# facebookresearch/Active-3D-Vision-and-Touch

Hardware: AMD Instinct MI355X
Metric: mesh-recon iters/sec (fwd+bwd, 2562-vert GCN + 10k-pt Chamfer) at bs=64 (higher is better)
Workload: dtype f32; 1 GPU; icosphere-4 template (2562 verts, 5120 faces), 3-stage GCN 20x300 cut 0.33, bs=64/GPU, 10000-pt Chamfer x3 draws, Adam, ellipsoid clouds (BASELINE.json configs[1]); global_batch=64, parallelism=dp1

## Files before the change

active-3d-vision-and-touch_amd/csrc/capi.hip:

```cpp
#include <stdarg.h>
#include <stdlib.h>
#include <string.h>

#include "../../include/a3vt.h"
#include <atomic>
#include <mutex>
#include <unordered_map>

#include "kernels.h"
#include "prims.h"

namespace a3vt {

static thread_local char g_err[512] = "";

void set_error(const char *fmt, ...) {
  va_list ap;
  va_start(ap, fmt);
  vsnprintf(g_err, sizeof(g_err), fmt, ap);
  va_end(ap);
}

__device__ float g_zero_page[64];
static const float *zero_page() {
// ... 35 lines not shown
static Prof g_prof;

struct ProfScope {
  int slot = -1;
  hipStream_t s;
  ProfScope(int cls, hipStream_t stream, bool timed = true) : s(stream) {
    if (!timed || !g_prof.on || g_prof.used >= Prof::kMax) return;
    slot = g_prof.used++;
    if (slot >= g_prof.created) {
      (void)hipEventCreate(&g_prof.ev[slot][0]);
      (void)hipEventCreate(&g_prof.ev[slot][1]);
      g_prof.created = slot + 1;
    }
    g_prof.cls[slot] = cls;
    (void)hipEventRecord(g_prof.ev[slot][0], s);
  }
  ~ProfScope() {
    if (slot >= 0) (void)hipEventRecord(g_prof.ev[slot][1], s);
  }
};

struct StackLayout {
  size_t wt, wt_stride;
  size_t za;
  int ldza;
  size_t z3;
  size_t ping[2];
  size_t panel;
  size_t dw_slab, db_slab, thin_dw_slab, thin_db_slab;
  size_t db_layer_stride;
  size_t heavy;
  size_t gq;
  size_t ell;
  size_t total;
};

constexpr int kQuadCols = 160;
static std::atomic<long long> g_path_counts[PATH_COUNT];
void path_count(int which) { g_path_counts[which].fetch_add(1, std::memory_order_relaxed); }
static int g_csr_algo = 0;
static SplitRef split_ref(const a3vt_adj_split *sp) {
  return sp ? SplitRef{sp->rowptr, sp->col, sp->scale, sp->cls} : SplitRef{nullptr, nullptr, nullptr, nullptr};
}
static bool split_whole(const a3vt_adj_split *sp) {
  const SplitRef r = split_ref(sp);
  return !sp || (r.rowptr && r.col && r.scale && r.cls);
}
static bool split_usable(const a3vt_adj_split *sp, int n_vert, int cut_len) {
  return sp && sp->max_degree > 0 && sp->max_degree <= csrqs_max_degree() && csrqs_fits(n_vert, cut_len);
}
static bool use_csrq(int batch, int n_vert, int hidden, int cut_len, int mode, int max_degree) {
  if (mode == GEMM_BF16_OPERANDS || mode == GEMM_BF16_STORAGE) return false;
  if (g_csr_algo != 2 && (max_degree <= 0 || max_degree > csrq_max_degree())) return false;
  if (g_csr_algo == 1 || cut_len <= 0) return false;
  return hidden % 4 == 0 && hidden >= kQuadCols + 16 && csrq_fits(n_vert, cut_len) && dw_quad_major_ok(hidden, kQuadCols / 4) &&
         rowgemm_quad_major_ok(batch * n_vert, hidden, pad4(cut_len));
}
static std::mutex g_stash_mu;
static std::unordered_map<const void *, int> g_stash_layout;
static void stash_layout_record(const void *masks, bool quad) {
  if (!masks) return;
  std::lock_guard<std::mutex> lock(g_stash_mu);
  if (g_stash_layout.size() > 4096) g_stash_layout.clear();
  g_stash_layout[masks] = quad ? 1 : 0;
}
static int stash_layout_lookup(const void *masks) {
  std::lock_guard<std::mutex> lock(g_stash_mu);
  auto it = g_stash_layout.find(masks);
  return it == g_stash_layout.end() ? -1 : it->second;
}
static int reduce_bias_partials(const float *slab, size_t layer_stride, int nslab, int cpad, int cut_len, int hidden, int last,
                                float *const *grad_biases, int acc, hipStream_t s) {
  for (int i0 = 0; i0 < last; i0 += kMaxImages) {
// ... 60 lines not shown
  bool x3;
  int omode;
  bool quad;
  bool qsplit;
  int qcols;
  int rm_ld;
  size_t rm_off;
};
static StackPlan stack_plan(int mode, int batch, int n_vert, int hidden, int num_layers, int cut_len, int max_degree,
                            const a3vt_adj_split *split, int rec) {
  StackPlan p{};
  const size_t m = (size_t)batch * n_vert;
  p.x3 = mode == GEMM_FP32X3 && num_layers > 2 && rowgemm3_stack_ok((long long)m, hidden, mask_ld(hidden, cut_len));
  p.omode = mode == GEMM_BF16_OPERANDS ? GEMM_BF16_OPERANDS : GEMM_FP32;
  const bool split_ok = split_usable(split, n_vert, cut_len);
  p.quad = num_layers > 1 &&
           (rec >= 0 ? rec == 1 : use_csrq(batch, n_vert, hidden, cut_len, mode, split_ok ? csrq_max_degree() : max_degree));
  p.qsplit = p.quad && split_ok;
  p.qcols = p.quad ? kQuadCols : 0;
  p.rm_ld = hidden - p.qcols;
  p.rm_off = m * p.qcols;
  return p;
}

static int launch_stack_ell(const StackPlan &p, const a3vt_adj_split *split, const int32_t *rowptr, const int32_t *col,
                            const float *val, int n_vert, int32_t *ell, hipStream_t s) {
  if (p.qsplit) {
    const SplitRef r = split_ref(split);
    return launch_csrqs_image(r.rowptr, r.col, r.scale, r.cls, n_vert, ell, s);
  }
  return p.quad ? launch_csrq_ell(rowptr, col, val, n_vert, ell, s) : 0;
}

static StackLayout stack_layout(int batch, int n_vert, int in_features, int hidden, int num_layers, int cut_len,
                                int need_backward, int gemm_mode = 0) {
  StackLayout L{};
  const size_t m = (size_t)batch * n_vert;
  const int cpad = pad4(cut_len);
  Arena a;
  const int kmax = hidden > pad4(in_features) ? hidden : pad4(in_features);
  L.wt_stride = align_up((size_t)rowgemm_bt_rows(kmax) * pad16(kmax), 64);
  if (gemm_mode == GEMM_FP32X3 && L.wt_stride < 3 * (size_t)kX3ImageFloats) L.wt_stride = 3 * (size_t)kX3ImageFloats;
  L.wt = a.take(L.wt_stride * (num_layers > 1 ? num_layers - 1 : 1));
  L.ldza = cpad > 4 ? cpad : 4;
  L.za = a.take(m * L.ldza);
  L.z3 = a.take(2 * m * 4);
  L.ping[0] = a.take(m * hidden);
  L.ping[1] = a.take(m * hidden);
  L.heavy = a.take(csr_heavy_scratch_ints(n_vert));
  L.ell = a.take(csrq_ell_ints(n_vert));
  if (need_backward) {
    const size_t kin = kmax;
    L.panel = a.take(pad4(in_features) > 304 ? m * 300 : 0);
    L.dw_slab = a.take((size_t)dw_slab_capacity(hidden) * kin * hidden);
    const size_t nslab = (size_t)csr_bwd_num_slabs(batch, n_vert) > (size_t)batch ? csr_bwd_num_slabs(batch, n_vert) : batch;
    L.db_layer_stride = align_up(nslab * cpad, 64);
    L.db_slab = a.take(L.db_layer_stride * (num_layers > 1 ? num_layers - 1 : 1));
    L.gq = a.take(m * L.ldza);
    L.thin_dw_slab = a.take((size_t)thin_num_slabs() * kin * 3);
    L.thin_db_slab = a.take((size_t)thin_num_slabs() * 3);
  }
  L.total = a.off;
  return L;
}

static int dw_panels(DwArgs d, const float *x, int ldx, int kin, float *panel, float *grad, int acc, bool timed, hipStream_t s) {
  const int cblk = kin > 304 ? 300 : kin;
  for (int c0 = 0; c0 < kin; c0 += cblk) {
    const int w = kin - c0 < cblk ? kin - c0 : cblk;
    d.x = x;
    d.ldx = ldx;
    if (kin > 304) {
      if (pad4(w) != w) { set_error("gcn_stack: in_features=%d needs a multiple of 4 past 300", kin); return -1; }
      if (int rc = launch_copy_cols(x, ldx, c0, w, panel, (long long)d.m, s)) return rc;
      d.x = panel;
      d.ldx = w;
    }
    d.k_in = w;
    {
      ProfScope ps(PROF_DW, s, timed);
      if (int rc = launch_dw(d, s)) return rc;
    }
    const size_t n = (size_t)w * d.n_out;
    if (int rc = launch_slab_reduce_za(d.slab, dw_images(d), n, n, n, grad + (size_t)c0 * d.n_out, acc, s)) return rc;
  }
  return 0;
}

static int check_stack_dims(int ld_feats, int in_features, int num_layers, int hidden, int cut_len) {
  if (num_layers < 1) { set_error("gcn_stack: num_layers=%d", num_layers); return -1; }
  if (ld_feats != pad4(in_features)) {
    set_error("gcn_stack: ld_feats=%d must be in_features=%d rounded up to a multiple of 4", ld_feats, in_features);
    return -1;
// ... 576 lines not shown
                           float *const *grad_biases, float *grad_feats, float *scratch, int accumulate, void *stream) {
  const int acc = accumulate ? 1 : 0;
  const float *acts = static_cast<const float *>(acts_v);
  (void)biases; (void)rowptr; (void)col; (void)val;
  A3VT_CHECK_ARG(feats && weights && rowptrT && colT && valT && grad_update && grad_weights && grad_biases);
  A3VT_CHECK_ARG(grad_feats && scratch && n_vert > 0 && batch > 0 && split_whole(split));
  A3VT_CHECK_ARG(gemm_bf16 >= GEMM_FP32 && gemm_bf16 <= GEMM_FP32X3);
  A3VT_CHECK_ARG(num_layers == 1 || acts != nullptr);
  A3VT_CHECK_ARG(num_layers <= 2 || masks != nullptr);
  if (int rc = check_stack_dims(ld_feats, in_features, num_layers, hidden, cut_len)) return rc;
  hipStream_t s = static_cast<hipStream_t>(stream);
  if (gemm_bf16 == GEMM_BF16_STORAGE)
    return stack_bwd16(feats, ld_feats, in_features, weights, num_layers, hidden, cut_len, rowptrT, colT, valT,
                       max_degreeT, split, n_vert, batch, acts, masks, grad_update, grad_weights, grad_biases, grad_feats,
                       scratch, acc, s);
  const float *zeros = zero_page();
  A3VT_CHECK_ARG(zeros != nullptr);
  const StackLayout L = stack_layout(batch, n_vert, in_features, hidden, num_layers, cut_len, 1, gemm_bf16);
  const StackStash S = stack_stash(batch, n_vert, hidden, num_layers, cut_len, gemm_bf16);
  const size_t m = (size_t)batch * n_vert;
  const int cpad = pad4(cut_len);
  const int last = num_layers - 1;

  const SplitRef sref = split_ref(split);
  int32_t *heavyT;
  if (int rc = hub_rows(rowptrT, n_vert, max_degreeT, scratch + L.heavy, &heavyT, s)) return rc;
  const StackPlan P = stack_plan(gemm_bf16, batch, n_vert, hidden, num_layers, cut_len, max_degreeT, split,
                                 masks ? stash_layout_lookup(masks) : 0);
  const bool quad = P.quad;
  const int qcols = P.qcols, rm_ld = P.rm_ld;
  const size_t rm_off = P.rm_off;
  int32_t *ellT = reinterpret_cast<int32_t *>(scratch + L.ell);
  if (int rc = launch_stack_ell(P, split, rowptrT, colT, valT, n_vert, ellT, s)) return rc;
  {
    const float *xl = num_layers == 1 ? feats : acts + S.act(last - 1);
    const float *x = xl + rm_off - qcols;
    const int ldx = num_layers == 1 ? ld_feats : rm_ld;
    const int k = num_layers == 1 ? in_features : hidden;
    float *gprev = num_layers == 1 ? grad_feats : scratch + L.ping[0];
    const int ldg = num_layers == 1 ? ld_feats : hidden;
    ProfScope pso(PROF_OUT, s);
    if (int rc = launch_thin_bwd(x, ldx, k, weights[last], rowptrT, colT, valT, heavyT, n_vert, batch, grad_update,
                                 scratch + L.z3, num_layers > 1, gprev, ldg, ldg, scratch + L.thin_dw_slab,
                                 scratch + L.thin_db_slab, quad ? scratch + L.gq : nullptr, cpad / 4, quad ? xl : nullptr,
                                 qcols / 4, s, split ? &sref : nullptr))
      return rc;
    if (int rc = reduce_output_grads(scratch + L.thin_dw_slab, scratch + L.thin_db_slab, k, grad_weights[last], grad_biases[last],
                                     acc, s))
      return rc;
  }

  if (P.x3)
    if (int rc = launch_stack_images(GEMM_FP32X3, 0, weights, 1, last, in_features, hidden, ld_feats, hidden, scratch + L.wt,
                                     L.wt_stride, s))
      return rc;
  if (int rc = launch_stack_images(GEMM_FP32, 0, weights, 0, P.x3 ? 1 : last, in_features, hidden, ld_feats, hidden,
                                   scratch + L.wt, L.wt_stride, s))
    return rc;

  const int db_rows = quad ? batch : csr_bwd_num_slabs(batch, n_vert);
  int cur = 0;
  for (int i = last - 1; i >= 0; --i) {
    float *g = scratch + L.ping[cur];
    float *dza = scratch + L.za;
    const float *xl = i == 0 ? feats : acts + S.act(i - 1);
    const bool xhyb = quad && i > 0;
    const float *x = xhyb ? xl + rm_off - qcols : xl;
    const int ldx = i == 0 ? ld_feats : (xhyb ? rm_ld : hidden);
    const int kin = i == 0 ? in_features : hidden;

    if (cut_len > 0 && quad) {
      const uint8_t *sq = masks + S.signq(i);
      ProfScope psa(PROF_AGG, s);
      if (P.qsplit) {
        if (int rc = launch_csrqs_bwd(scratch + L.gq, cut_len, ellT, n_vert, batch, dza, sq,
                                      scratch + L.db_slab + (size_t)i * L.db_layer_stride, s))
          return rc;
      } else if (int rc = launch_csrq_bwd(scratch + L.gq, cut_len, rowptrT, colT, valT, heavyT, ellT, n_vert, batch, dza, sq,
                                          scratch + L.db_slab + (size_t)i * L.db_layer_stride, s)) {
        return rc;
      }
    } else if (cut_len > 0) {
      ProfScope psa(PROF_AGG, s);
      if (int rc = launch_csr_bwd(g, hidden, cut_len, rowptrT, colT, valT, heavyT, n_vert, batch, dza, L.ldza,
                                  scratch + L.db_slab + (size_t)i * L.db_layer_stride, s))
        return rc;
    } else if (!acc) {
      if (int rc = launch_fill_zero(grad_biases[i], hidden, s)) return rc;
    }

    DwArgs d{};
    if (xhyb) {
      d.ldx_src = rm_ld;
      d.xq = xl;
      d.xq_nvert = n_vert;
      d.xq_quads = qcols / 4;
    }
    if (quad) {
      d.z0q_nvert = n_vert;
      d.z0q_quads = cpad / 4;
    }
    d.z0 = dza;
    d.ldz0 = L.ldza;
    d.z1 = g;
    d.ldz1 = hidden;
    d.zsplit = cpad;
    d.zeros = zeros;
    d.slab = scratch + L.dw_slab;
    d.m = (int)m;
    d.n_out = hidden;
    d.mode = P.omode;
    const int ldxw = xhyb ? hidden : ldx;
    if (P.x3 && i > 0) {
      d.mode = GEMM_FP32X3;
      d.x = x;
      d.ldx = ldxw;
      d.k_in = kin;
      if (!dw3_ok(d)) d.mode = P.omode;
    }
    if (int rc = dw_panels(d, x, ldxw, kin, scratch + L.panel, grad_weights[i], acc, true, s)) return rc;

    RowGemmArgs r{};
    r.a0 = dza;
    r.lda0 = L.ldza;
    if (quad) {
      r.a0q_nvert = n_vert;
      r.a0q_quads = cpad / 4;
    }
    r.a1 = g;
    r.lda1 = hidden;
    r.ksplit = cpad;
    r.bt = scratch + L.wt + L.wt_stride * i;
    r.ldb = pad16(hidden);
    r.zeros = zeros;
    r.m = (int)m;
    r.k = hidden;
    r.n_store = i == 0 ? ld_feats : hidden;
    r.mode = P.x3 && i > 0 ? GEMM_FP32X3 : P.omode;
    if (i == 0) {
      r.c = grad_feats;
      r.ldc = ld_feats;
      if (int rc = launch_rowgemm(r, EPI_PLAIN, s)) return rc;
    } else {
      r.c = scratch + L.ping[cur ^ 1];
      r.ldc = hidden;
      r.maskb = const_cast<uint8_t *>(masks) + S.signs(i - 1);
      r.mld = S.mld;
      r.moff = cpad / 4;
      r.csplit = cut_len;
      if (quad) {
        r.c2 = scratch + L.gq;
        r.zq_nvert = n_vert;
        r.zq_quads = cpad / 4;
        r.trash = scratch + L.z3;
      }
      {
        ProfScope ps(PROF_GEMM_DX, s);
        if (int rc = launch_rowgemm(r, EPI_DX_MASK, s)) return rc;
      }
      cur ^= 1;
    }
  }
  if (cut_len > 0)
    if (int rc = reduce_bias_partials(scratch + L.db_slab, L.db_layer_stride, db_rows, cpad, cut_len, hidden, last, grad_biases, acc, s))
      return rc;
  return 0;
}

namespace {
struct LayerLayout {
  size_t wt, za, ga, dz, panel, dw_slab, db_slab, heavy, total;
  int ldza;
};
LayerLayout layer_layout(int batch, int n_vert, int ld_x, int n_out, int cut_len, int need_backward) {
  LayerLayout L{};
  const size_t m = (size_t)batch * n_vert;
  const int cpad = pad4(cut_len), npad = pad4(n_out);
// ... 1038 lines not shown
  g_prof.on = on != 0;
  g_prof.used = 0;
  return 0;
}

int a3vt_profile_read_classes(double *total_ms, int *count, int n) {
  A3VT_CHECK_ARG(total_ms && count && n >= 0);
  for (int c = 0; c < n; ++c) { total_ms[c] = 0.0; count[c] = 0; }
  for (int i = 0; i < g_prof.used; ++i) {
    if (hipEventSynchronize(g_prof.ev[i][1]) != hipSuccess) { set_error("profile_read: event sync failed"); return -2; }
    float ms = 0.f;
    if (hipEventElapsedTime(&ms, g_prof.ev[i][0], g_prof.ev[i][1]) != hipSuccess) continue;
    if (g_prof.cls[i] >= n) continue;
    total_ms[g_prof.cls[i]] += ms;
    count[g_prof.cls[i]] += 1;
  }
  g_prof.used = 0;
  return PROF_CLASSES;
}

int a3vt_profile_read(double *total_ms, int *count) {
  const int rc = a3vt_profile_read_classes(total_ms, count, 3);
  return rc < 0 ? rc : 0;
}

int a3vt_dbg_path_counts(long long *counts, int n, int reset) {
  A3VT_CHECK_ARG(n >= 0 && (counts != nullptr || n == 0));
  for (int i = 0; i < n; ++i) counts[i] = i < PATH_COUNT ? g_path_counts[i].load(std::memory_order_relaxed) : 0;
  if (reset)
    for (auto &c : g_path_counts) c.store(0, std::memory_order_relaxed);
  return PATH_COUNT;
}

int a3vt_dbg_csr_algo(int algo) {
  A3VT_CHECK_ARG(algo >= 0 && algo <= 2);
  g_csr_algo = algo;
  return 0;
}

int a3vt_split3_bf16(const float *x, size_t n, uint16_t *hi, uint16_t *mid, uint16_t *lo, void *stream) {
  A3VT_CHECK_ARG(n == 0 || (x && hi && mid && lo));
  return launch_split3(x, n, hi, mid, lo, static_cast<hipStream_t>(stream));
}

int a3vt_check_finite(const float *data, size_t n, int32_t *flag, void *stream) {
  A3VT_CHECK_ARG(data && flag);
  return launch_check_finite(data, n, flag, static_cast<hipStream_t>(stream));
}

}
```

active-3d-vision-and-touch_amd/csrc/common.h:

```cpp
#pragma once
#include <hip/hip_runtime.h>
#include <stdint.h>
#include <stdio.h>

#include <mutex>

namespace a3vt {

void set_error(const char *fmt, ...);

#define A3VT_CHECK_ARG(cond)                                                              \
  do {                                                                                    \
    if (!(cond)) {                                                                        \
      a3vt::set_error("%s:%d: argument check failed: %s", __FILE__, __LINE__, #cond);     \
      return -1;                                                                          \
    }                                                                                     \
  } while (0)

#define A3VT_LAUNCH(...)            \
  do {                              \
    (void)hipGetLastError();        \
    hipLaunchKernelGGL(__VA_ARGS__); \
  } while (0)

// ... 8 lines not shown
  } while (0)

struct OncePerDevice {
  std::mutex mu;
  unsigned long long done = 0;
  template <class F>
  void run(F &&f) {
    int dev = 0;
    (void)hipGetDevice(&dev);
    const unsigned long long bit = 1ull << (dev & 63);
    std::lock_guard<std::mutex> lock(mu);
    if (!(done & bit)) {
      f();
      done |= bit;
    }
  }
};

enum PathCount {
  PATH_STACK_QUAD = 0,
  PATH_STACK_ROWS,
  PATH_RG_ADIRECT,
  PATH_RG3,
  PATH_DW3,
  PATH_DW_HYBRID,
  PATH_RG16,
  PATH_STACK16_QUAD,
  PATH_RGW,
  PATH_DWW,
  PATH_STACK_SPLIT,
  PATH_CSR16T,
  PATH_QNET_FWD,
  PATH_QNET_BWD,
  PATH_FOLD_FWD,
  PATH_FOLD_BWD,
  PATH_COUNT
};
void path_count(int which);

__host__ __device__ static inline int cdiv(long long a, long long b) { return (int)((a + b - 1) / b); }
__host__ __device__ static inline int pad4(int n) { return (n + 3) & ~3; }
__host__ __device__ static inline int pad8(int n) { return (n + 7) & ~7; }
__host__ __device__ static inline int pad16(int n) { return (n + 15) & ~15; }
static inline bool aligned_to(const void *p, unsigned bytes) { return (reinterpret_cast<uintptr_t>(p) & (bytes - 1)) == 0; }

constexpr int kWave = 64;

struct FixScale {
  int shift;
};
__device__ __forceinline__ FixScale fix_scale(float bound, long long count) {
  int e = 0;
  (void)frexpf(bound, &e);
  int c = 1;
  while ((1ll << c) <= count) ++c;
  return FixScale{62 - e - c};
}
__device__ __forceinline__ long long fix_from(float t, FixScale s) { return __float2ll_rn(ldexpf(t, s.shift)); }
__device__ __forceinline__ float fix_to(long long a, FixScale s) { return ldexpf((float)a, -s.shift); }
__device__ __forceinline__ void fix_add(long long *acc, long long v) {
  atomicAdd(reinterpret_cast<unsigned long long *>(acc), (unsigned long long)v);
}

}
```

active-3d-vision-and-touch_amd/csrc/gcn_dww.hip:

```cpp
#include <type_traits>

#include "gemm_tile.h"

namespace a3vt {

constexpr int kDK = 300, kDN = 300, kDXQ = 40, kDZQ = 25, kDXRW = 140, kDLdz = 300;
constexpr int kDStageRows = 16;
constexpr int kDwwGroupsA = 135, kDwwGroupsB = 121;
constexpr int kDXQ_off = 0, kDXR_off = 2560, kDZ_off = 2560 + 2304;
constexpr int kDZRa_off = kDZ_off + 1792;
constexpr int kDStage = kDZ_off + 2816;
constexpr int kDStages = 4;
constexpr int kDLdsFloats = kDStages * kDStage;

__device__ __forceinline__ void d_mfma(f32x4 &acc, float a, float b) {
  asm volatile("v_mfma_f32_16x16x4_f32 %0, %1, %2, %0" : "+a"(acc) : "v"(a), "v"(b));
}
__device__ __forceinline__ void d_lds(float &dst, unsigned base, int imm) {
  asm volatile("ds_read_b32 %0, %1 offset:%2" : "=v"(dst) : "v"(base), "n"(imm));
}
template <int N, int NX, int NZ>
__device__ __forceinline__ void d_wait(float (&x)[NX], float (&z)[NZ]) {
  static_assert(NX <= 5 && NZ <= 10, "operand list");
  if constexpr (NX == 5 && NZ == 10)
// ... 179 lines not shown
      if (k < kDK && col < kDN) *reinterpret_cast<f32x4 *>(img + (size_t)k * kDN + col) = acc[t][n];
    }
  }
}

__global__ __launch_bounds__(256) __attribute__((amdgpu_waves_per_eu(1, 1))) void dww_kernel(DwArgs p) {
  extern __shared__ __attribute__((aligned(16))) float lds[];
  const int lane = threadIdx.x & 63;
  const int wave = __builtin_amdgcn_readfirstlane(threadIdx.x >> 6);
  const int half = blockIdx.x < kDwwGroupsA ? 0 : 1;
  const int group = half == 0 ? blockIdx.x : blockIdx.x - kDwwGroupsA, ngroups = half == 0 ? kDwwGroupsA : kDwwGroupsB;
  const int tiles = p.m / kDStageRows;
  const int t0 = (int)((long long)group * tiles / ngroups), t1 = (int)((long long)(group + 1) * tiles / ngroups);
  if (half == 1 && group < kDwwGroupsA - kDwwGroupsB) {
    float *img = p.slab + (size_t)(kDwwGroupsB + group) * kDK * kDN;
    for (int i = threadIdx.x; i < kDK * 35; i += 256) {
      const int k = i / 35, c = i - k * 35;
      *reinterpret_cast<f32x4 *>(img + (size_t)k * kDN + 160 + c * 4) = f32x4{0.f, 0.f, 0.f, 0.f};
    }
  }
  if (half == 0) {
    if (wave == 0) dww_wave<0, false, 5, false, 0>(p, lds, lane, t0, t1, group);
    else if (wave == 1) dww_wave<0, false, 5, false, 5>(p, lds, lane, t0, t1, group);
    else if (wave == 2) dww_wave<0, true, 5, false, 10>(p, lds, lane, t0, t1, group);
    else dww_wave<0, true, 4, true, 15>(p, lds, lane, t0, t1, group);
  } else {
    if (wave == 0) dww_wave<1, false, 5, false, 0>(p, lds, lane, t0, t1, group);
    else if (wave == 1) dww_wave<1, false, 5, false, 5>(p, lds, lane, t0, t1, group);
    else if (wave == 2) dww_wave<1, true, 5, false, 10>(p, lds, lane, t0, t1, group);
    else dww_wave<1, true, 4, true, 15>(p, lds, lane, t0, t1, group);
  }
}

bool dww_ok(const DwArgs &a) {
  if (a.mode != GEMM_FP32 || a.xq_nvert <= 0 || a.z0q_nvert != a.xq_nvert || a.xq == nullptr) return false;
  if (a.k_in != kDK || a.n_out != kDN || a.xq_quads != kDXQ || a.z0q_quads != kDZQ || a.zsplit != 4 * kDZQ) return false;
  if (a.ldx_src != kDXRW || a.ldz1 != kDLdz || a.m % a.xq_nvert != 0 || a.m % kDStageRows != 0 || a.xq_nvert < 16) return false;
  if (a.m > 3000000) return false;
  return a.m / kDStageRows >= kDwwGroupsA * 5;
}

int dww_images() { return kDwwGroupsA; }

int launch_dww(const DwArgs &a, hipStream_t s) {
  if (!dww_ok(a)) {
    set_error("dww: shape not taken (m=%d k_in=%d n_out=%d)", a.m, a.k_in, a.n_out);
    return -1;
  }
  static OncePerDevice once;
  once.run([] {
    (void)hipFuncSetAttribute((const void *)dww_kernel, hipFuncAttributeMaxDynamicSharedMemorySize, (int)(kDLdsFloats * sizeof(float)));
  });
  path_count(PATH_DWW);
  A3VT_LAUNCH(dww_kernel, dim3(kDwwGroupsA + kDwwGroupsB), dim3(256), kDLdsFloats * sizeof(float), s, a);
  A3VT_CHECK_LAUNCH();
  return 0;
}

}
```

active-3d-vision-and-touch_amd/csrc/kernels.h:

```cpp
#pragma once
#include <hip/hip_runtime.h>
#include <stddef.h>
#include <stdint.h>

namespace a3vt {

enum { EPI_PLAIN = 0, EPI_FWD_HIDDEN = 1, EPI_DX_MASK = 2 };
enum GemmMode { GEMM_FP32 = 0, GEMM_BF16_OPERANDS = 1, GEMM_BF16_STORAGE = 2, GEMM_FP32X3 = 3 };

struct RowGemmArgs {
  const float *a0;
  const float *a1;
  const float *bt;
  const float *zeros;
  uint8_t *maskb;
  float *c;
  float *c2;
  int lda0, lda1, ksplit, ldb;
  int bt_rows;
  int col0;
  int m, k, n_store;
  int ldc, ldc2, csplit, mld, moff;
  int no_relu;
  int plain_relu;
// ... 35 lines not shown
constexpr int kX3ImageLd = 160;
constexpr int kX3ImageFloats = kX3ImageRows * kX3ImageLd;
bool rowgemm3_dims_ok(long long m, int k, int n_store);
bool rowgemm3_stack_ok(long long m, int hidden, int mld);
bool rowgemm3_ok(const RowGemmArgs &a, int epi);
int launch_rowgemm3(const RowGemmArgs &a, int epi, hipStream_t s);
int launch_weight_images3(const WeightImages &w, hipStream_t s);
int launch_split3(const float *x, size_t n, unsigned short *hi, unsigned short *mid, unsigned short *lo, hipStream_t s);

struct DwArgs {
  const float *x;
  const float *z0;
  const float *z1;
  const float *zeros;
  float *slab;
  int ldx, ldz0, ldz1, zsplit;
  int m, k_in, n_out;
  int mode;
  int nstage;
  const float *xq;
  int ldx_src, xq_nvert, xq_quads, z0q_nvert, z0q_quads;
};
int dw_num_slabs(int n_out);
int dw_images(const DwArgs &a);
int dw_slab_capacity(int n_out);
bool dw3_ok(const DwArgs &a);
int launch_dw3(const DwArgs &a, hipStream_t s);
bool dw_quad_major_ok(int k_in, int quads);
bool dw_rows_fit(int ldx, int ldz0, int ldz1);
int launch_dw(const DwArgs &a, hipStream_t s);
bool dww_ok(const DwArgs &a);
int dww_images();
int launch_dww(const DwArgs &a, hipStream_t s);
int launch_copy_cols(const float *src, int ld_src, int c0, int w, float *dst, long long m, hipStream_t s);
int launch_slab_reduce(const float *slab, int nslab, size_t stride, size_t n, float *out, hipStream_t s);
int launch_slab_reduce_za(const float *slab, int nslab, size_t stride, size_t n, size_t n_out, float *out, int accumulate,
                          hipStream_t s);

int launch_csr_fwd(const float *za, int ldza, const float *bias, int c, const int32_t *rowptr, const int32_t *col,
                   const float *val, const int32_t *heavy, int n_vert, int batch, float *y, int ldy, uint8_t *maskb,
                   int mld, int relu, hipStream_t s);
size_t csr_heavy_scratch_ints(int n_vert);
int csr_heavy_degree();
int launch_csr_heavy_list(const int32_t *rowptr, int n_vert, int32_t *heavy, hipStream_t s);
int launch_relu_split(const float *gy, int ldgy, const float *y, int ldy, int relu, int n_out, int cpad, int npad,
                      long long m, float *ga, float *dz, hipStream_t s);
int csr_bwd_num_slabs(int batch, int n_vert);
int launch_csr_bwd(const float *g, int ldg, int c, const int32_t *rowptrT, const int32_t *colT, const float *valT,
                   const int32_t *heavyT, int n_vert, int batch, float *dza, int lddza, float *db_slab, hipStream_t s);

bool csrq_fits(int n_vert, int cut_len);
int csrq_max_degree();
size_t csrq_ell_ints(int n_vert);
int launch_csrq_ell(const int32_t *rowptr, const int32_t *col, const float *val, int n_vert, int32_t *ell, hipStream_t s);
int launch_csrq_fwd(const float *zq, const float *bias, int c, const int32_t *rowptr, const int32_t *col,
                    const float *val, const int32_t *heavy, const int32_t *ell, int n_vert, int batch, float *yq,
                    int yq_quads ,
                    uint8_t *signq, int relu, hipStream_t s);
int launch_csrq_bwd(const float *gq, int c, const int32_t *rowptrT, const int32_t *colT, const float *valT,
                    const int32_t *heavyT, const int32_t *ellT, int n_vert, int batch, float *dzaq, const uint8_t *signq,
                    float *db_slab, hipStream_t s);
struct SplitRef {
  const int32_t *rowptr, *col;
  const float *scale;
  const uint8_t *cls;
};
// ... 255 lines not shown
```

active-3d-vision-and-touch_amd/lib.py:

```python
import ctypes
import os
import subprocess

_HERE = os.path.dirname(os.path.abspath(__file__))
CSRC = os.path.join(_HERE, "csrc")
LIB_PATH = os.environ.get("A3VT_LIB", os.path.join(_HERE, "liba3vt.so"))
SOURCES = ["capi.hip", "gcn_gemm.hip", "gcn_gemmw.hip", "gcn_dww.hip", "gcn_gemm16.hip", "gcn_gemm3.hip", "gcn_csr.hip", "gcn_csrq.hip", "gcn_csrqs.hip", "gcn_bf16s.hip", "posenc.hip", "posenc_wide.hip", "bias_grad.hip", "bnrelu.hip", "conv5.hip", "conv5f.hip", "adam.hip", "sample.hip", "chamfer.hip", "nn_prune.hip",
           "pooling.hip", "fold.hip", "ddqn.hip", "qnet_input.hip", "latent_nn.hip", "latent_policy.hip", "ddqn_latent.hip",
           "candidate_tally.hip", "touch_render.hip"]
EXTRA_FLAGS = {"chamfer.hip": ["-fno-slp-vectorize"], "nn_prune.hip": ["-fno-slp-vectorize"],
               "gcn_csrq.hip": ["-fno-slp-vectorize"], "gcn_csrqs.hip": ["-fno-slp-vectorize"],
               "gcn_gemmw.hip": ["-std=c++20"], "gcn_dww.hip": ["-std=c++20"]}

_vp, _i, _sz, _u64, _f = ctypes.c_void_p, ctypes.c_int, ctypes.c_size_t, ctypes.c_uint64, ctypes.c_float


class AdjSplit(ctypes.Structure):
    _fields_ = [("rowptr", _vp), ("col", _vp), ("scale", _vp), ("cls", _vp),
                ("max_degree", ctypes.c_int32), ("n_seam", ctypes.c_int32), ("n_centre", ctypes.c_int32)]


class MlpLayer(ctypes.Structure):
    _fields_ = [("weight", _vp), ("bias", _vp), ("n_in", ctypes.c_int32), ("n_out", ctypes.c_int32), ("relu", ctypes.c_int32),
                ("reserved", ctypes.c_int32)]
# ... 77 lines not shown
    "a3vt_chamfer_workspace_bytes": (_sz, [_i, _i, _i, _i]),
    "a3vt_chamfer_fwd_ws": (_i, [_vp, _vp, _i, _i, _i, _i, _vp, _vp, _vp, _vp, _vp, _vp, _sz, _i, _vp]),
    "a3vt_chamfer_fwd_shared": (_i, [_vp, _vp, _i, _i, _i, _i, _i, _vp, _vp, _vp, _vp, _vp, _vp, _sz, _i, _vp]),
    "a3vt_chamfer_bwd": (_i, [_vp, _vp, _i, _i, _i, _i, _vp, _vp, _vp, _vp, _vp, _vp]),
    "a3vt_fold_workspace_bytes": (_sz, [_i, _i, _i]),
    "a3vt_fold_fwd": (_i, [_vp, _vp, _i, _vp, _vp, _vp, _vp, _vp, _i, _i, _i, _vp, _vp, _sz, _vp]),
    "a3vt_fold_bwd": (_i, [_vp, _vp, _i, _vp, _vp, _vp, _vp, _vp, _i, _i, _i, _vp, _vp, _vp, _vp, _vp, _vp, _vp, _vp, _sz, _vp]),
    "a3vt_ddqn_td": (_i, [_vp, _vp, _vp, _vp, _vp, _vp, _vp, _i, _i, _i, ctypes.c_float, _vp, _vp, _vp, _vp, _vp]),
    "a3vt_ddqn_td_bwd": (_i, [_vp, _vp, _vp, _i, _i, _vp, _vp]),
    "a3vt_latent_nearest_scratch_bytes": (_sz, [_i, _i, _i]),
    "a3vt_latent_nearest": (_i, [_vp, _vp, _i, _i, _vp, _vp, _i, _i, _i, _vp, _vp, _vp, _vp, _vp, _vp]),
    "a3vt_latent_nn_tile": (_i, []),
    "a3vt_latent_nn_query_floats": (_i, []),
    "a3vt_latent_nn_cached_rows": (_i, []),
    "a3vt_candidate_tally": (_i, [_vp, _vp, _vp, _vp, _i, _i, _i, ctypes.c_double, _vp, _vp, _vp, _vp, _vp, _vp]),
    "a3vt_touch_render": (_i, [_vp, _i, _vp, _i, _vp, _i, _vp, _vp, _vp, _i, _f, _f, _f, _f, _vp, _vp, _vp, _vp, _vp, _vp]),
    "a3vt_touch_finish": (_i, [_vp, _vp, _vp, _i, _f, _f, _vp, _vp, _vp, _vp, _vp]),
    "a3vt_latent_policy_limit": (_i, [_i]),
    "a3vt_latent_policy_stash_floats": (_i, [_vp]),
    "a3vt_latent_policy_fwd": (_i, [_vp, _vp, _vp, _vp, _vp, _i, _vp, _vp, _vp, _vp]),
    "a3vt_action_value_loss": (_i, [_vp, _vp, _vp, _i, _i, _i, _vp, _vp, _vp]),
    "a3vt_latent_policy_bwd": (_i, [_vp, _vp, _vp, _vp, _vp, _vp, _vp, _vp, _i, _i, _vp]),
    "a3vt_latent_policy_launches": (_i, [_vp, _i]),
    "a3vt_ddqn_latent_scratch_bytes": (_sz, [_vp, _i]),
    "a3vt_ddqn_latent_q": (_i, [_vp, _vp, _vp, _vp, _vp, _i, _vp, _vp, _vp]),
    "a3vt_ddqn_latent_update": (_i, [_vp, _vp, _vp, _vp, _vp, _vp, _vp, _vp, _vp, _vp, _vp, _i, _i, ctypes.c_float,
                                     _vp, _vp, _vp, _vp, _vp, _vp, _vp]),
    "a3vt_ddqn_latent_launches": (_i, [_vp, _i]),
    "a3vt_qnet_input_scratch_bytes": (_sz, [_i, _i, _i, _i, _i]),
    "a3vt_qnet_input_fwd": (_i, [_vp, _vp, _vp, _vp, _vp, _vp, _vp, _vp, _vp, _i, _i, _vp, _vp, _vp, _i, _i, _i, _vp, _i, _vp, _vp]),
    "a3vt_qnet_input_bwd": (_i, [_vp, _vp, _vp, _vp, _vp, _vp, _i, _i, _vp, _vp, _vp, _i, _i, _i, _vp, _i, _vp, _i,
                                 _vp, _vp, _vp, _vp, _vp, _vp, _vp, _vp, _vp, _vp]),
    "a3vt_dbg_csr_algo": (_i, [_i]),
    "a3vt_dbg_path_counts": (_i, [_vp, _i, _i]),
    "a3vt_dbg_nn_work": (_i, [_i, _vp]),
    "a3vt_split3_bf16": (_i, [_vp, _sz, _vp, _vp, _vp, _vp]),
    "a3vt_check_finite": (_i, [_vp, _sz, _vp, _vp]),
    "a3vt_profile_enable": (_i, [_i]),
    "a3vt_profile_read": (_i, [_vp, _vp]),
    "a3vt_profile_read_classes": (_i, [_vp, _vp, _i]),
}

_LIB = None


def build(force=False, verbose=False):
    return _build(force, verbose, LIB_PATH, os.path.join(_HERE, "build"))


def _build(force, verbose, lib_path, objdir):
    srcs = [os.path.join(CSRC, s) for s in SOURCES]
    deps = srcs + [os.path.join(CSRC, h) for h in ("common.h", "kernels.h", "prims.h", "policy_dev.h", "gemm_tile.h")] + \
        [os.path.join(_HERE, "..", "include", "a3vt.h")]
    force = force or os.environ.get("A3VT_FORCE_BUILD", "0") not in ("", "0")
    if not force and os.path.exists(lib_path) and all(
            os.path.getmtime(lib_path) >= os.path.getmtime(d) for d in deps if os.path.exists(d)):
        return lib_path
    hipcc = os.environ.get("HIPCC", "/opt/rocm/bin/hipcc")
    if not os.path.exists(hipcc):
        hipcc = "hipcc"
    common = ["-O3", "--offload-arch=gfx950", "-std=c++17", "-fPIC"]
    os.makedirs(objdir, exist_ok=True)
    procs = []
    for name in SOURCES:
        obj = os.path.join(objdir, name.replace(".hip", ".o"))
        cmd = [hipcc, *common, *EXTRA_FLAGS.get(name, []), "-c", os.path.join(CSRC, name), "-o", obj]
# ... 41 lines not shown
```

active-3d-vision-and-touch_amd/ops.py:

```python
import ctypes
import weakref

import numpy as np
import torch

from . import lib as _lib
from .mesh import CSRAdjacency


def _stream():
    return ctypes.c_void_p(torch.cuda.current_stream().cuda_stream)


def _req(t, name, dtype=torch.float32):
    if not isinstance(t, torch.Tensor) or not t.is_cuda:
        raise RuntimeError(f"a3vt: `{name}` must be a tensor on the GPU (the HIP path has no CPU fallback)")
    if t.dtype != dtype:
        raise RuntimeError(f"a3vt: `{name}` must be {dtype}, got {t.dtype}")
    return t.contiguous()


_WORKSPACES = {}
STATS = {"stack_calls": 0, "stack_stash_calls": 0}

# ... 19 lines not shown
        self.host = host
        self.max_degree = int(np.diff(host.rowptr).max()) if host.n else 0
        self.t_max_degree = int(np.diff(host.t_rowptr).max()) if host.n else 0
        self.split = self.split_struct = None
        sp = host.split() if self.max_degree > 8 else None
        if sp is not None:
            _lib.check(L.a3vt_adj_split_validate(host.rowptr.ctypes.data, host.col.ctypes.data, host.val.ctypes.data, host.n,
                                                 sp.rowptr.ctypes.data, sp.col.ctypes.data, sp.scale.ctypes.data,
                                                 sp.cls.ctypes.data), "adj_split_validate")
            self.split = (to(sp.rowptr), to(sp.col), to(sp.scale), to(sp.cls))
            self.split_struct = _lib.AdjSplit(*[t.data_ptr() for t in self.split], sp.max_degree, sp.n_seam, sp.n_centre)
        self.use_split = True

    def split_ref(self):
        return ctypes.byref(self.split_struct) if (self.split_struct is not None and self.use_split) else None

    @property
    def device(self):
        return self.val.device


def _wants_grad(*tensors):
    return torch.is_grad_enabled() and any(t.requires_grad for t in tensors)


def _ptr_array(tensors):
    return (ctypes.c_void_p * len(tensors))(*[t.data_ptr() for t in tensors])


GEMM_MODES = {"fp32": 0, "bf16": 1, "bf16s": 2, "fp32x3": 3}


PATH_NAMES = ("stack_quad", "stack_rows", "rowgemm_adirect", "rowgemm3", "dw3", "dw_hybrid", "rowgemm16", "stack16_quad", "rowgemm_w", "dw_w", "stack_split", "csr16_tiles",
              "qnet_input_fwd", "qnet_input_bwd", "fold_fwd", "fold_bwd")


def path_counts(reset=False):
    import ctypes
    buf = (ctypes.c_longlong * len(PATH_NAMES))()
    _lib.load().a3vt_dbg_path_counts(buf, len(PATH_NAMES), 1 if reset else 0)
    return dict(zip(PATH_NAMES, (int(x) for x in buf)))


def nn_work(enable):
    import ctypes
    buf = (ctypes.c_ulonglong * 8)()
    _lib.check(_lib.load().a3vt_dbg_nn_work(1 if enable else 0, buf), "dbg_nn_work")
    names = ("waves", "groups", "blocks", "box_tests", "max_groups_per_wave")
    return dict(zip(names, (int(x) for x in buf)))


def gemm_mode(bf16):
    if isinstance(bf16, str):
        return GEMM_MODES[bf16]
    return int(bf16)


class GradSink:
    __slots__ = ("view", "written", "expect", "on_final")

    def __init__(self, view, on_final=None):
        self.view, self.written, self.expect, self.on_final = view, False, 0, on_final

    def reset(self):
        self.written, self.expect = False, 0


# ... 1476 lines not shown
def qnet_input(mesh, action, pos_enc, mask_table, weight, bias, adj, cut_len):
    l1, l2, l3 = pos_enc.model[0], pos_enc.model[2], pos_enc.model[4]
    wa, wp, wm = weight[:100], weight[100:200], weight[200:300]
    comp_s = torch.addmm(l3.bias @ wp, action, wa)
    comp_t = mask_table @ wm
    comp_c = l3.weight.t() @ wp
    pad = (-weight.shape[1]) % 4
    if pad:
        comp_s, comp_t, comp_c = (torch.nn.functional.pad(t, (0, pad)) for t in (comp_s, comp_t, comp_c))
    params = (l1.weight, l1.bias, l2.weight, l2.bias, comp_s, comp_t, comp_c, bias)
    return QnetInputFn.apply(mesh, *params, adj, cut_len, _wants_grad(*params))


def rowgemm(a, w, bf16=False):
    L = _lib.load()
    a, w = _req(a, "a"), _req(w, "w")
    M, K = a.shape
    N = w.shape[1]
    wt = torch.empty((L.a3vt_wt_rows(N), L.a3vt_wt_ld(K)), dtype=torch.float32, device=a.device)
    _lib.check(L.a3vt_transpose_weight(_lib.ptr(w), K, N, _lib.ptr(wt), _stream()), "transpose_weight")
    c = torch.empty((M, N), dtype=torch.float32, device=a.device)
    _lib.check(L.a3vt_rowgemm(_lib.ptr(a), K, M, K, _lib.ptr(wt), N, 1 if bf16 else 0, _lib.ptr(c), N, _stream()),
               "rowgemm")
    return c


CSR_ALGOS = {"auto": 0, "rows": 1, "sliced": 2}


def dbg_csr_algo(name):
    _lib.check(_lib.load().a3vt_dbg_csr_algo(CSR_ALGOS[name]), "dbg_csr_algo")


def split3(x):
    L = _lib.load()
    x = _req(x, "x")
    hi, mid, lo = (torch.empty(x.shape, dtype=torch.int16, device=x.device) for _ in range(3))
    _lib.check(L.a3vt_split3_bf16(_lib.ptr(x), x.numel(), _lib.ptr(hi), _lib.ptr(mid), _lib.ptr(lo), _stream()), "split3_bf16")
    return hi, mid, lo


def check_finite(t, flag):
    L = _lib.load()
    _lib.check(L.a3vt_check_finite(_lib.ptr(t), t.numel(), _lib.ptr(flag), _stream()), "check_finite")
```

include/a3vt.h:

```cpp
#ifndef A3VT_H
#define A3VT_H
#include <stddef.h>
#include <stdint.h>

#ifdef __cplusplus
extern "C" {
#endif

#define A3VT_VERSION 163

int a3vt_version(void);
const char *a3vt_last_error(void);

int a3vt_csr_validate(const int32_t *rowptr_host, const int32_t *col_host, int n_vert, int nnz);

size_t a3vt_gcn_stack_scratch_bytes(int batch, int n_vert, int in_features, int hidden, int num_layers,
                                    int cut_len, int need_backward);
size_t a3vt_gcn_stack_mask_bytes(int batch, int n_vert, int hidden, int num_layers, int cut_len);
size_t a3vt_gcn_stack_scratch_bytes_mode(int batch, int n_vert, int in_features, int hidden, int num_layers,
                                         int cut_len, int need_backward, int gemm_bf16);
int a3vt_gcn_stack_stash_bytes(int batch, int n_vert, int hidden, int num_layers, int cut_len, int gemm_bf16,
                               size_t *acts_bytes, size_t *mask_bytes);

int a3vt_gcn_stack_fwd(const float *feats, int ld_feats, int in_features,
// ... 140 lines not shown
                         const int *chunk_tensor, const long long *chunk_off, int n_chunks, double lr, double beta1, double beta2,
                         double eps, double weight_decay, long long step, double grad_clamp, void *stream);

int a3vt_vertex_update(const float *verts_in, const float *update, int batch, int n_vert, int n_vision,
                       float *verts_out, void *stream);

int a3vt_face_cdf(const float *verts, const int32_t *faces, int batch, int n_vert, int n_faces,
                  float *cdf, void *stream);
int a3vt_sample_points_fwd(const float *verts, const int32_t *faces, const float *cdf,
                           int batch, int n_vert, int n_faces, int draws, int num,
                           const int32_t *face_idx_in, const float *u_in, const float *v_in,
                           uint64_t seed, uint64_t offset,
                           float *points, int32_t *face_idx_out, float *u_out, float *v_out, void *stream);
int a3vt_sample_points_bwd(const int32_t *faces, int batch, int n_vert, int n_faces, int draws, int num,
                           const int32_t *face_idx, const float *u, const float *v,
                           const float *grad_points, float *grad_verts, void *stream);

size_t a3vt_chamfer_scratch_bytes(int draws, int batch, int p, int q);
int a3vt_chamfer_fwd(const float *x, const float *y, int draws, int batch, int p, int q,
                     float *dist_xy, int32_t *idx_xy, float *dist_yx, int32_t *idx_yx, float *cd,
                     void *scratch, void *stream);
size_t a3vt_chamfer_workspace_bytes(int draws, int batch, int p, int q);
int a3vt_chamfer_fwd_ws(const float *x, const float *y, int draws, int batch, int p, int q,
                        float *dist_xy, int32_t *idx_xy, float *dist_yx, int32_t *idx_yx, float *cd,
                        void *workspace, size_t workspace_bytes, int algo, void *stream);
int a3vt_chamfer_fwd_shared(const float *x, const float *y, int draws, int batch, int y_batch, int p, int q,
                            float *dist_xy, int32_t *idx_xy, float *dist_yx, int32_t *idx_yx, float *cd,
                            void *workspace, size_t workspace_bytes, int algo, void *stream);
int a3vt_chamfer_bwd(const float *x, const float *y, int draws, int batch, int p, int q,
                     const int32_t *idx_xy, const int32_t *idx_yx, const float *grad_cd,
                     float *grad_x, float *grad_y, void *stream);

int a3vt_dbg_csr_algo(int algo);

int a3vt_dbg_path_counts(long long *counts, int n, int reset);

int a3vt_dbg_nn_work(int enable, unsigned long long *out8);

int a3vt_split3_bf16(const float *x, size_t n, uint16_t *hi, uint16_t *mid, uint16_t *lo, void *stream);

size_t a3vt_fold_workspace_bytes(int batch, int points, int backward);
int a3vt_fold_fwd(const float *bias_s, const float *g, int k, const float *w1g, const float *w2, const float *b2, const float *w3,
                  const float *b3, int batch, int points, int width, float *y, void *workspace, size_t workspace_bytes, void *stream);
int a3vt_fold_bwd(const float *bias_s, const float *g, int k, const float *w1g, const float *w2, const float *b2, const float *w3,
                  const float *dy, int batch, int points, int width, float *d_bias_s, float *dg, float *dw1g, float *dw2, float *db2,
                  float *dw3, float *db3, void *workspace, size_t workspace_bytes, void *stream);

int a3vt_ddqn_td(const float *q_cur, const float *q_next_online, const float *q_next_target, const float *mask, const float *actions,
                 const float *rewards, const float *denom, int batch, int num_actions, int budget, float gamma, float *loss,
                 float *diff, int32_t *best_next, float *target, void *stream);
int a3vt_ddqn_td_bwd(const float *diff, const float *actions, const float *grad_loss, int batch, int num_actions, float *dq_cur,
                     void *stream);

size_t a3vt_latent_nearest_scratch_bytes(int n_queries, int bank_rows, int k);
int a3vt_latent_nearest(const float *bank, const int32_t *bank_actions, int bank_rows, int dim, const float *queries, const float *taken,
                        int n_queries, int num_actions, int k, int32_t *idx, float *dist, int32_t *action, int32_t *rank, void *scratch,
                        void *stream);
int a3vt_latent_nn_tile(void);
int a3vt_latent_nn_query_floats(void);
int a3vt_latent_nn_cached_rows(void);

int a3vt_candidate_tally(const float *scores, const int32_t *candidates, const float *first_score, const float *taken, int K, int E, int A,
                         double unvisited, double *sums, double *checks, double *votes, int32_t *best, float *best_score, void *stream);

int a3vt_touch_render(const float *verts, int V, const int32_t *faces, int F, const int32_t *face_offset, int M, const int32_t *image_mesh,
                      const float *cam_pos, const float *cam_rot, int I, float max_depth, float yfov, float znear, float zfar, float *depth,
// ... 57 lines not shown
```

Measured before the change: 21.93 iters/s.

## Batch weight-gradient GEMMs of several GCN layers into one stacked kernel launch

```diff
diff --git a/active-3d-vision-and-touch_amd/csrc/capi.hip b/active-3d-vision-and-touch_amd/csrc/capi.hip
--- a/active-3d-vision-and-touch_amd/csrc/capi.hip
+++ b/active-3d-vision-and-touch_amd/csrc/capi.hip
@@ -91,6 +91,8 @@
   size_t heavy;
   size_t gq;
   size_t ell;
+  size_t keep, keep_za, keep_stride;
+  int keep_slots;
   size_t total;
 };
 
@@ -98,6 +100,8 @@
 static std::atomic<long long> g_path_counts[PATH_COUNT];
 void path_count(int which) { g_path_counts[which].fetch_add(1, std::memory_order_relaxed); }
 static int g_csr_algo = 0;
+constexpr size_t kDwKeepBudgetBytes = (size_t)6 << 30;
+static int g_dw_defer = 0;
 static SplitRef split_ref(const a3vt_adj_split *sp) {
   return sp ? SplitRef{sp->rowptr, sp->col, sp->scale, sp->cls} : SplitRef{nullptr, nullptr, nullptr, nullptr};
 }
@@ -224,6 +228,20 @@
   return p.quad ? launch_csrq_ell(rowptr, col, val, n_vert, ell, s) : 0;
 }
 
+static inline size_t keep_g_floats(size_t m, int hidden) { return align_up(m * hidden, 64); }
+static int dw_defer_window(int gemm_mode, int batch, int n_vert, int hidden, int num_layers, int cut_len) {
+  const size_t m = (size_t)batch * n_vert;
+  const int deferrable = num_layers - 2;
+  if (gemm_mode != GEMM_FP32 || g_dw_defer == 1 || deferrable < 2 || hidden != 300 || pad4(cut_len) != 100) return 1;
+  if (!dww_rows_ok((long long)m, n_vert)) return 1;
+  const size_t slot = (keep_g_floats(m, hidden) + align_up(m * pad4(cut_len), 64)) * sizeof(float);
+  size_t w = kDwKeepBudgetBytes / slot;
+  w = w < (size_t)deferrable ? w : (size_t)deferrable;
+  w = w < (size_t)kMaxImages ? w : (size_t)kMaxImages;
+  if (g_dw_defer > 1 && w > (size_t)g_dw_defer) w = g_dw_defer;
+  return w < 2 ? 1 : (int)w;
+}
+
 static StackLayout stack_layout(int batch, int n_vert, int in_features, int hidden, int num_layers, int cut_len,
                                 int need_backward, int gemm_mode = 0) {
   StackLayout L{};
@@ -244,13 +262,25 @@
   if (need_backward) {
     const size_t kin = kmax;
     L.panel = a.take(pad4(in_features) > 304 ? m * 300 : 0);
-    L.dw_slab = a.take((size_t)dw_slab_capacity(hidden) * kin * hidden);
+    size_t dw_images = dw_slab_capacity(hidden);
+    const int window = dw_defer_window(gemm_mode, batch, n_vert, hidden, num_layers, cut_len);
+    if (window > 1) {
+      L.keep_slots = window;
+      const size_t need = (size_t)window * dww_images();
+      dw_images = need > dw_images ? need : dw_images;
+    }
+    L.dw_slab = a.take(dw_images * kin * hidden);
     const size_t nslab = (size_t)csr_bwd_num_slabs(batch, n_vert) > (size_t)batch ? csr_bwd_num_slabs(batch, n_vert) : batch;
     L.db_layer_stride = align_up(nslab * cpad, 64);
     L.db_slab = a.take(L.db_layer_stride * (num_layers > 1 ? num_layers - 1 : 1));
     L.gq = a.take(m * L.ldza);
     L.thin_dw_slab = a.take((size_t)thin_num_slabs() * kin * 3);
     L.thin_db_slab = a.take((size_t)thin_num_slabs() * 3);
+    if (L.keep_slots > 0) {
+      L.keep_za = keep_g_floats(m, hidden);
+      L.keep_stride = L.keep_za + align_up(m * L.ldza, 64);
+      L.keep = a.take(L.keep_stride * L.keep_slots);
+    }
   }
   L.total = a.off;
   return L;
@@ -893,12 +923,32 @@
   const size_t rm_off = P.rm_off;
   int32_t *ellT = reinterpret_cast<int32_t *>(scratch + L.ell);
   if (int rc = launch_stack_ell(P, split, rowptrT, colT, valT, n_vert, ellT, s)) return rc;
+  const int window = L.keep_slots;
+  bool defer = window > 1 && quad && P.omode == GEMM_FP32 && !P.x3;
+  if (defer) {
+    DwArgs probe{};
+    probe.mode = GEMM_FP32;
+    probe.xq = acts;
+    probe.xq_nvert = probe.z0q_nvert = n_vert;
+    probe.xq_quads = qcols / 4;
+    probe.z0q_quads = cpad / 4;
+    probe.zsplit = cpad;
+    probe.ldx_src = rm_ld;
+    probe.ldz1 = hidden;
+    probe.m = (int)m;
+    probe.k_in = probe.n_out = hidden;
+    defer = dww_ok(probe);
+  }
+  auto slot_of = [&](int i) { return (last - 1 - i) % window; };
+  auto slot_g = [&](int j) { return scratch + L.keep + (size_t)j * L.keep_stride; };
+  auto slot_za = [&](int j) { return scratch + L.keep + (size_t)j * L.keep_stride + L.keep_za; };
+  DwwStackArgs dws{};
   {
     const float *xl = num_layers == 1 ? feats : acts + S.act(last - 1);
     const float *x = xl + rm_off - qcols;
     const int ldx = num_layers == 1 ? ld_feats : rm_ld;
     const int k = num_layers == 1 ? in_features : hidden;
-    float *gprev = num_layers == 1 ? grad_feats : scratch + L.ping[0];
+    float *gprev = num_layers == 1 ? grad_feats : (defer ? slot_g(0) : scratch + L.ping[0]);
     const int ldg = num_layers == 1 ? ld_feats : hidden;
     ProfScope pso(PROF_OUT, s);
     if (int rc = launch_thin_bwd(x, ldx, k, weights[last], rowptrT, colT, valT, heavyT, n_vert, batch, grad_update,
@@ -922,8 +972,9 @@
   const int db_rows = quad ? batch : csr_bwd_num_slabs(batch, n_vert);
   int cur = 0;
   for (int i = last - 1; i >= 0; --i) {
-    float *g = scratch + L.ping[cur];
-    float *dza = scratch + L.za;
+    const bool kept = defer && i > 0;
+    float *g = kept ? slot_g(slot_of(i)) : scratch + L.ping[cur];
+    float *dza = kept ? slot_za(slot_of(i)) : scratch + L.za;
     const float *xl = i == 0 ? feats : acts + S.act(i - 1);
     const bool xhyb = quad && i > 0;
     const float *x = xhyb ? xl + rm_off - qcols : xl;
@@ -979,7 +1030,31 @@
       d.k_in = kin;
       if (!dw3_ok(d)) d.mode = P.omode;
     }
-    if (int rc = dw_panels(d, x, ldxw, kin, scratch + L.panel, grad_weights[i], acc, true, s)) return rc;
+    if (kept) {
+      const int n = dws.layers++;
+      dws.layer[n] = DwwLayer{xl, x, dza, g};
+      dws.out[n] = grad_weights[i];
+      if (slot_of(i) == window - 1 || i == 1) {
+        if (dws.layers == 1) {
+          if (int rc = dw_panels(d, x, ldxw, kin, scratch + L.panel, grad_weights[i], acc, true, s)) return rc;
+        } else {
+          dws.shape = d;
+          dws.shape.x = dws.shape.xq = dws.shape.z0 = dws.shape.z1 = nullptr;
+          dws.shape.ldx = ldxw;
+          dws.shape.k_in = kin;
+          dws.shape.xq = xl;
+          dws.accumulate = acc;
+          {
+            ProfScope ps(PROF_DW, s);
+            if (int rc = launch_dww_stack(dws, s)) return rc;
+          }
+          if (int rc = launch_dww_stack_reduce(dws, s)) return rc;
+        }
+        dws.layers = 0;
+      }
+    } else if (int rc = dw_panels(d, x, ldxw, kin, scratch + L.panel, grad_weights[i], acc, true, s)) {
+      return rc;
+    }
 
     RowGemmArgs r{};
     r.a0 = dza;
@@ -1003,7 +1078,7 @@
       r.ldc = ld_feats;
       if (int rc = launch_rowgemm(r, EPI_PLAIN, s)) return rc;
     } else {
-      r.c = scratch + L.ping[cur ^ 1];
+      r.c = defer && i > 1 ? slot_g(slot_of(i - 1)) : scratch + L.ping[cur ^ 1];
       r.ldc = hidden;
       r.maskb = const_cast<uint8_t *>(masks) + S.signs(i - 1);
       r.mld = S.mld;
@@ -2108,6 +2183,29 @@
   return PATH_COUNT;
 }
 
+int a3vt_dbg_dw_defer(int max_layers) {
+  if (max_layers < 0 || max_layers > kMaxImages) { set_error("dbg_dw_defer: max_layers=%d (0..%d)", max_layers, kMaxImages); return -1; }
+  g_dw_defer = max_layers;
+  return 0;
+}
+
+int a3vt_dw_defer_plan(int tiles, int layers, int half, int group, int layer, int *segment, int *images_per_layer) {
+  if (tiles < 1 || layers < 1 || layers > kMaxImages || half < 0 || half > 1 || group < 0 || group >= dww_stack_groups(half) ||
+      layer < 0 || layer >= layers || tiles < dww_stack_groups(0)) {
+    set_error("dw_defer_plan: tiles=%d layers=%d half=%d group=%d layer=%d", tiles, layers, half, group, layer);
+    return -1;
+  }
+  const DwwSegment seg = dww_stack_plan(tiles, half, group, layer);
+  if (segment) {
+    segment[0] = seg.layer;
+    segment[1] = seg.t0;
+    segment[2] = seg.t1;
+    segment[3] = seg.image;
+  }
+  if (images_per_layer) *images_per_layer = dww_images();
+  return 1;
+}
+
 int a3vt_dbg_csr_algo(int algo) {
   A3VT_CHECK_ARG(algo >= 0 && algo <= 2);
   g_csr_algo = algo;
diff --git a/active-3d-vision-and-touch_amd/csrc/common.h b/active-3d-vision-and-touch_amd/csrc/common.h
--- a/active-3d-vision-and-touch_amd/csrc/common.h
+++ b/active-3d-vision-and-touch_amd/csrc/common.h
@@ -64,6 +64,7 @@
   PATH_CSR16T,
   PATH_QNET_FWD,
   PATH_QNET_BWD,
+  PATH_DWW_STACK,
   PATH_FOLD_FWD,
   PATH_FOLD_BWD,
   PATH_COUNT
diff --git a/active-3d-vision-and-touch_amd/csrc/gcn_dww.hip b/active-3d-vision-and-touch_amd/csrc/gcn_dww.hip
--- a/active-3d-vision-and-touch_amd/csrc/gcn_dww.hip
+++ b/active-3d-vision-and-touch_amd/csrc/gcn_dww.hip
@@ -235,6 +235,92 @@
   }
 }
 
+__global__ __launch_bounds__(256) __attribute__((amdgpu_waves_per_eu(1, 1))) void dww_stack_kernel(DwwStackArgs a) {
+  extern __shared__ __attribute__((aligned(16))) float lds[];
+  const int lane = threadIdx.x & 63;
+  const int wave = __builtin_amdgcn_readfirstlane(threadIdx.x >> 6);
+  const int half = blockIdx.x < kDwwGroupsA ? 0 : 1;
+  const int group = half == 0 ? blockIdx.x : blockIdx.x - kDwwGroupsA, ngroups = half == 0 ? kDwwGroupsA : kDwwGroupsB;
+  const int tiles = a.shape.m / kDStageRows;
+  const int t0 = (int)((long long)group * tiles / ngroups), t1 = (int)((long long)(group + 1) * tiles / ngroups);
+  for (int layer = 0; layer < a.layers; ++layer) {
+    if (layer > 0) {
+      if (wave == 3) wait_vmcnt<0>();
+      wait_lgkm0();
+      __builtin_amdgcn_s_barrier();
+    }
+    DwArgs p = a.shape;
+    p.xq = a.layer[layer].xq;
+    p.x = a.layer[layer].x;
+    p.z0 = a.layer[layer].z0;
+    p.z1 = a.layer[layer].z1;
+    p.slab = a.shape.slab + (size_t)layer * kDwwGroupsA * kDK * kDN;
+    if (half == 1 && group < kDwwGroupsA - kDwwGroupsB) {
+      float *img = p.slab + (size_t)(kDwwGroupsB + group) * kDK * kDN;
+      for (int i = threadIdx.x; i < kDK * 35; i += 256) {
+        const int k = i / 35, c = i - k * 35;
+        *reinterpret_cast<f32x4 *>(img + (size_t)k * kDN + 160 + c * 4) = f32x4{0.f, 0.f, 0.f, 0.f};
+      }
+    }
+    if (half == 0) {
+      if (wave == 0) dww_wave<0, false, 5, false, 0>(p, lds, lane, t0, t1, group);
+      else if (wave == 1) dww_wave<0, false, 5, false, 5>(p, lds, lane, t0, t1, group);
+      else if (wave == 2) dww_wave<0, true, 5, false, 10>(p, lds, lane, t0, t1, group);
+      else dww_wave<0, true, 4, true, 15>(p, lds, lane, t0, t1, group);
+    } else {
+      if (wave == 0) dww_wave<1, false, 5, false, 0>(p, lds, lane, t0, t1, group);
+      else if (wave == 1) dww_wave<1, false, 5, false, 5>(p, lds, lane, t0, t1, group);
+      else if (wave == 2) dww_wave<1, true, 5, false, 10>(p, lds, lane, t0, t1, group);
+      else dww_wave<1, true, 4, true, 15>(p, lds, lane, t0, t1, group);
+    }
+  }
+}
+
+bool dww_rows_ok(long long m, int n_vert) {
+  if (m <= 0 || n_vert < 16 || m % n_vert != 0 || m % kDStageRows != 0) return false;
+  if (m > 3000000) return false;
+  return m / kDStageRows >= kDwwGroupsA * 5;
+}
+
+int dww_stack_groups(int half) { return half == 0 ? kDwwGroupsA : kDwwGroupsB; }
+
+DwwSegment dww_stack_plan(int tiles, int half, int group, int layer) {
+  const int n = dww_stack_groups(half);
+  return DwwSegment{layer, (int)((long long)group * tiles / n), (int)((long long)(group + 1) * tiles / n), group};
+}
+
+static bool dww_stack_args_ok(const DwwStackArgs &a) {
+  if (a.layers >= 1 && a.layers <= kMaxImages && dww_ok(a.shape)) return true;
+  set_error("dww_stack: not taken (layers=%d m=%d)", a.layers, a.shape.m);
+  return false;
+}
+
+int launch_dww_stack(const DwwStackArgs &a, hipStream_t s) {
+  if (!dww_stack_args_ok(a)) return -1;
+  static OncePerDevice once;
+  once.run([] {
+    (void)hipFuncSetAttribute((const void *)dww_stack_kernel, hipFuncAttributeMaxDynamicSharedMemorySize, (int)(kDLdsFloats * sizeof(float)));
+  });
+  for (int l = 0; l < a.layers; ++l) path_count(PATH_DWW);
+  path_count(PATH_DWW_STACK);
+  A3VT_LAUNCH(dww_stack_kernel, dim3(kDwwGroupsA + kDwwGroupsB), dim3(256), kDLdsFloats * sizeof(float), s, a);
+  A3VT_CHECK_LAUNCH();
+  return 0;
+}
+
+int launch_dww_stack_reduce(const DwwStackArgs &a, hipStream_t s) {
+  if (!dww_stack_args_ok(a)) return -1;
+  SlabReduceBatch b{};
+  b.count = a.layers;
+  b.slab = a.shape.slab;
+  for (int l = 0; l < a.layers; ++l) b.out[l] = a.out[l];
+  b.layer_stride = (size_t)kDwwGroupsA * kDK * kDN;
+  b.stride = b.n = b.n_out = (size_t)kDK * kDN;
+  b.nslab = kDwwGroupsA;
+  b.accumulate = a.accumulate;
+  return launch_slab_reduce_batch(b, s);
+}
+
 bool dww_ok(const DwArgs &a) {
   if (a.mode != GEMM_FP32 || a.xq_nvert <= 0 || a.z0q_nvert != a.xq_nvert || a.xq == nullptr) return false;
   if (a.k_in != kDK || a.n_out != kDN || a.xq_quads != kDXQ || a.z0q_quads != kDZQ || a.zsplit != 4 * kDZQ) return false;
diff --git a/active-3d-vision-and-touch_amd/csrc/kernels.h b/active-3d-vision-and-touch_amd/csrc/kernels.h
--- a/active-3d-vision-and-touch_amd/csrc/kernels.h
+++ b/active-3d-vision-and-touch_amd/csrc/kernels.h
@@ -91,6 +91,23 @@
 bool dww_ok(const DwArgs &a);
 int dww_images();
 int launch_dww(const DwArgs &a, hipStream_t s);
+struct DwwLayer {
+  const float *xq, *x, *z0, *z1;
+};
+struct DwwStackArgs {
+  DwArgs shape;
+  DwwLayer layer[kMaxImages];
+  float *out[kMaxImages];
+  int layers, accumulate;
+};
+struct DwwSegment {
+  int layer, t0, t1, image;
+};
+bool dww_rows_ok(long long m, int n_vert);
+int dww_stack_groups(int half);
+DwwSegment dww_stack_plan(int tiles, int half, int group, int layer);
+int launch_dww_stack(const DwwStackArgs &a, hipStream_t s);
+int launch_dww_stack_reduce(const DwwStackArgs &a, hipStream_t s);
 int launch_copy_cols(const float *src, int ld_src, int c0, int w, float *dst, long long m, hipStream_t s);
 int launch_slab_reduce(const float *slab, int nslab, size_t stride, size_t n, float *out, hipStream_t s);
 int launch_slab_reduce_za(const float *slab, int nslab, size_t stride, size_t n, size_t n_out, float *out, int accumulate,
diff --git a/active-3d-vision-and-touch_amd/lib.py b/active-3d-vision-and-touch_amd/lib.py
--- a/active-3d-vision-and-touch_amd/lib.py
+++ b/active-3d-vision-and-touch_amd/lib.py
@@ -133,6 +133,8 @@
     "a3vt_qnet_input_bwd": (_i, [_vp, _vp, _vp, _vp, _vp, _vp, _i, _i, _vp, _vp, _vp, _i, _i, _i, _vp, _i, _vp, _i,
                                  _vp, _vp, _vp, _vp, _vp, _vp, _vp, _vp, _vp, _vp]),
     "a3vt_dbg_csr_algo": (_i, [_i]),
+    "a3vt_dbg_dw_defer": (_i, [_i]),
+    "a3vt_dw_defer_plan": (_i, [_i, _i, _i, _i, _i, _vp, _vp]),
     "a3vt_dbg_path_counts": (_i, [_vp, _i, _i]),
     "a3vt_dbg_nn_work": (_i, [_i, _vp]),
     "a3vt_split3_bf16": (_i, [_vp, _sz, _vp, _vp, _vp, _vp]),
diff --git a/active-3d-vision-and-touch_amd/ops.py b/active-3d-vision-and-touch_amd/ops.py
--- a/active-3d-vision-and-touch_amd/ops.py
+++ b/active-3d-vision-and-touch_amd/ops.py
@@ -75,7 +75,7 @@
 
 
 PATH_NAMES = ("stack_quad", "stack_rows", "rowgemm_adirect", "rowgemm3", "dw3", "dw_hybrid", "rowgemm16", "stack16_quad", "rowgemm_w", "dw_w", "stack_split", "csr16_tiles",
-              "qnet_input_fwd", "qnet_input_bwd", "fold_fwd", "fold_bwd")
+              "qnet_input_fwd", "qnet_input_bwd", "dw_w_stack", "fold_fwd", "fold_bwd")
 
 
 def path_counts(reset=False):
@@ -1618,6 +1618,10 @@
     _lib.check(_lib.load().a3vt_dbg_csr_algo(CSR_ALGOS[name]), "dbg_csr_algo")
 
 
+def dbg_dw_defer(max_layers):
+    _lib.check(_lib.load().a3vt_dbg_dw_defer(int(max_layers)), "dbg_dw_defer")
+
+
 def split3(x):
     L = _lib.load()
     x = _req(x, "x")
diff --git a/include/a3vt.h b/include/a3vt.h
--- a/include/a3vt.h
+++ b/include/a3vt.h
@@ -196,6 +196,9 @@
                      float *grad_x, float *grad_y, void *stream);
 
 int a3vt_dbg_csr_algo(int algo);
+
+int a3vt_dbg_dw_defer(int max_layers);
+int a3vt_dw_defer_plan(int tiles, int layers, int half, int group, int layer, int *segment, int *images_per_layer);
 
 int a3vt_dbg_path_counts(long long *counts, int n, int reset);
 
```

Result: no change. 22.05 iters/s, median of 6 (+0.6%).
